# EllarBooher/Syzygy

Hardware: AMD Instinct MI355X
Metric: Mpixels/s deferred-lit+atmosphere (higher is better)
Workload: dtype f32

## Files before the change

syzygy_amd/_lib.py:

```python
import ctypes
import os
import sys

from . import abi

_HERE = os.path.dirname(os.path.abspath(__file__))
_LIB = None


class SzgError(RuntimeError):

    def __init__(self, code, message):
        super().__init__(f"szg status {code}: {message}")
        self.code = code


def library_path():
    return os.environ.get("SZG_HIP_LIBRARY") or os.path.join(_HERE, "csrc", "libszg_hip.so")


def lib():
    global _LIB
    if _LIB is None:
        path = library_path()
        if not os.path.exists(path):
            raise RuntimeError(
                f"{path} is missing: build it with `python -c 'import __graft_entry__ as g; g.build()'` "
                "(or `make -C syzygy_amd/csrc`). There is no CPU fallback for this path."
            )
        import torch

        handle = ctypes.CDLL(path)
        handle.szg_abi_version.restype = ctypes.c_int
        handle.szg_abi_version.argtypes = []
        version = handle.szg_abi_version()
        if version != abi.SZG_ABI_VERSION:
            raise RuntimeError(f"{path}: ABI version {version}, this package needs {abi.SZG_ABI_VERSION}; rebuild the library")
        abi.bind(handle, abi.ABI_FUNCTIONS)
        abi.bind(handle, abi.HOST_FUNCTIONS)
        abi.bind(handle, abi.RASTER_FUNCTIONS)
        abi.bind(handle, abi.ASSET_FUNCTIONS)
        abi.bind(handle, abi.DEBUGLINE_FUNCTIONS)
        try:
            abi.bind(handle, abi.PRESENT_FUNCTIONS)
        except AttributeError as e:
            raise RuntimeError(f"{path} predates include/szg/present.h ({e}); rebuild the library") from e
        try:
            abi.bind(handle, abi.COMPUTE_COLLECTION_FUNCTIONS)
        except AttributeError as e:
            raise RuntimeError(f"{path} predates include/szg/compute_collection.h ({e}); rebuild the library") from e
        try:
            abi.bind(handle, abi.MIPMAP_FUNCTIONS)
        except AttributeError as e:
            if "SZG_HIP_LIBRARY" not in os.environ:
                raise RuntimeError(f"{path} predates include/szg/mipmaps.h ({e}); rebuild the library") from e
            print(f"[szg] {path} predates include/szg/mipmaps.h ({e}): mip-mapped textures are unavailable with it", file=sys.stderr)
        _LIB = handle
    return _LIB


def check(status):
    if status != abi.SZG_OK:
        raise SzgError(status, lib().szg_last_error().decode("utf-8", "replace"))
    return status
```

syzygy_amd/abi.py:

```python
import ctypes as C

import numpy as np

SZG_ABI_VERSION = 2

SZG_OK = 0
SZG_ERR_INVALID_ARGUMENT = -1
SZG_ERR_NO_DEVICE = -2
SZG_ERR_OUT_OF_MEMORY = -3
SZG_ERR_HIP = -4
SZG_ERR_CAPACITY = -5

SZG_AERIAL_W = SZG_AERIAL_H = SZG_AERIAL_D = 32
SZG_OETF_PURE_GAMMA = 0
SZG_OETF_SRGB = 1

SZG_ROWTILE_COMM_ID_BYTES = 256
SZG_LUT_TRANSMITTANCE = 1
SZG_LUT_SKYVIEW = 2
SZG_FORMAT_UNDEFINED = 0
SZG_FORMAT_RGBA16_SFLOAT = 1
SZG_FORMAT_RGBA32_SFLOAT = 2
SZG_FORMAT_RGBA16_UNORM = 3
SZG_FORMAT_D32_SFLOAT = 4
# ... 481 lines not shown
    "szg_debug_lines_box_transform": (None, [P(Transform), P(AABB), P(VertexPacked)]),
}

SZG_DEBUG_LINES_CAPACITY = 1000
SZG_DEBUG_LINES_DEFAULT_WIDTH = 1.0
SZG_DEBUG_LINES_MAX_WIDTH = 256.0
SZG_DEBUG_LINES_GUARD_BAND = 16777216.0
SZG_DEBUG_LINES_MAX_CAPACITY = 1 << 24

DEBUGLINE_FUNCTIONS = {
    "szg_debug_lines_create": (C.c_int, [P(VP), U32, C.c_int]),
    "szg_debug_lines_destroy": (None, [VP]),
    "szg_debug_lines_record": (C.c_int, [VP, VP, C.c_float, Rect, P(RowTile), P(SceneTexture), U32, VP, VP, U32]),
}

SZG_PRESENT_MAX_EXTENT = 16384
SZG_FILTER_NEAREST = 0
SZG_FILTER_LINEAR = 1
SZG_PRESENT_ENCODE_NONE = 0xFFFFFFFF


class PresentInfo(C.Structure):
    _fields_ = [("src_region", Rect), ("dst_region", Rect), ("filter", U32), ("encode", U32)]


PRESENT_FUNCTIONS = {
    "szg_record_present": (C.c_int, [VP, P(Image), P(Image), P(PresentInfo)]),
}

SZG_COMPUTE_COLLECTION_SHADER_COUNT = 4
SZG_COMPUTE_COLLECTION_MAX_EXTENT = 16384
SZG_COMPUTE_COLLECTION_MAX_BLOCK_BYTES = 208
SZG_COMPUTE_COLLECTION_PREFIX_BYTES = 16
SZG_COMPUTE_COLLECTION_MAX_MEMBERS = 6
SZG_COMPUTE_COLLECTION_WORKGROUP = 16
SZG_CC_BOOLEANPUSH = 0
SZG_CC_GRADIENT_COLOR = 1
SZG_CC_SPARSE_PUSH_CONSTANT = 2
SZG_CC_MATRIX_COLOR = 3
SZG_CC_COMPONENT_FLOAT = 0
SZG_CC_COMPONENT_BOOL = 1


class CCMember(C.Structure):
    _fields_ = [("name", C.c_char_p), ("offset_bytes", U32), ("size_bytes", U32), ("padded_size_bytes", U32),
                ("component_type", U32), ("vector_width", U32), ("column_count", U32)]


class CCReflection(C.Structure):
    _fields_ = [("name", C.c_char_p), ("size_bytes", U32), ("padded_size_bytes", U32), ("layout_offset_bytes", U32),
                ("local_size", U32 * 3), ("member_count", U32), ("members", CCMember * SZG_COMPUTE_COLLECTION_MAX_MEMBERS)]


COMPUTE_COLLECTION_EXAMPLE_VALUES = {
    "booleanpush": {"row1": [1, 0, 1, 0], "row2": [0, 1, 0, 1], "row3": [1, 0, 1, 0], "row4": [0, 1, 0, 1]},
    "gradient_color": {"topColor": [0.05, 0.10, 0.60, 1.0], "bottomColor": [1.0, 0.55, 0.10, 1.0]},
    "sparse_push_constant": {"topRG": [0.9, 0.2], "topBA": [0.3, 1.0], "bottomRG": [0.1, 0.8], "bottomBA": [0.6, 1.0]},
    "matrix_color": {"red": [c / 3.0 for c in range(4) for _ in range(4)],
                     "green": [r / 3.0 for _ in range(4) for r in range(4)],
                     "blue": [((r + c) % 2) * 0.75 for c in range(4) for r in range(4)]},
}

COMPUTE_COLLECTION_FUNCTIONS = {
    "szg_compute_collection_shader_count": (U32, []),
    "szg_compute_collection_reflect": (C.c_int, [U32, P(CCReflection)]),
    "szg_record_compute_collection": (C.c_int, [VP, U32, VP, U32, P(Image), U32, U32]),
}

SZG_SAMPLER_MAX_LOD_REFERENCE = 1.0
SZG_SAMPLER_MAX_LOD_NONE = 1000.0


class TextureMips(C.Structure):
    _fields_ = [("level0_data", VP), ("d_chain", VP), ("level_count", U32)]


MIPMAP_FUNCTIONS = {
    "szg_mip_level_count": (U32, [U32, U32]),
    "szg_mip_chain_bytes": (C.c_size_t, [U32, U32]),
    "szg_record_generate_mipmaps": (C.c_int, [VP, P(Texture), VP, C.c_size_t]),
    "szg_deferred_set_texture_mips": (C.c_int, [VP, P(TextureMips), U32, C.c_float]),
}


def bind(lib, table):
    for name, (restype, argtypes) in table.items():
        fn = getattr(lib, name)
        fn.restype = restype
        fn.argtypes = argtypes
    return lib
```

syzygy_amd/csrc/api_skyview.cpp:

```cpp

#include <new>

#include "api_common.hpp"
#include "lut_state.hpp"

using namespace szg;

struct szg_skyview
{
    int device = 0;
    szg_skyview_desc desc{};
    DeviceBuffer<float> d_transmittance, d_skyview, d_multiscatter, d_aerialLuminance, d_aerialTransmittance;
    float aerialMaxDistance = 0.0f;
    mutable LutState luts;
    DeviceBuffer<unsigned> d_slutStatusAll;
    bool lutReuse = false;
    DeviceBuffer<unsigned> d_lutKey;
    DeviceBuffer<void> d_framePrep;
    DeviceBuffer<void> d_framePrepDraw;
};

static hipError_t ensure_tlut_status(szg_skyview* p, hipStream_t s)
{
    hipError_t e = hipSuccess;
    p->luts.ensure_tlut_status([&] {
        e = launch_lut_range(s, p->d_transmittance, p->desc.transmittance_width, p->desc.transmittance_height);
        return e == hipSuccess;
    });
    return e;
}

static hipError_t ensure_slut_status(szg_skyview* p, hipStream_t s)
{
    hipError_t e = hipSuccess;
    p->luts.ensure_slut_status([&] {
        e = launch_slut_check(s, p->d_skyview, p->desc.skyview_width, p->desc.skyview_height);
        return e == hipSuccess;
    });
    return e;
}

extern "C" {

int szg_skyview_create(szg_skyview_t** out, const szg_skyview_desc* desc, int device)
{
    if (out == nullptr)
    {
        return fail(SZG_ERR_INVALID_ARGUMENT, "szg_skyview_create: out is NULL");
    }
    *out = nullptr;
    szg_skyview_desc d{512u, 128u, 2048u, 1024u, 0u, 0u};
    if (desc != nullptr)
    {
        d = *desc;
    }
    if (d.transmittance_width < 2u || d.transmittance_height < 2u || d.skyview_width < 2u || d.skyview_height < 2u ||
        d.transmittance_width > 16384u || d.transmittance_height > 16384u || d.skyview_width > 16384u ||
        d.skyview_height > 16384u)
    {
        return fail(SZG_ERR_INVALID_ARGUMENT, "szg_skyview_create: LUT extents out of range");
    }
    if (d.flags != 0u)
    {
        return fail(SZG_ERR_INVALID_ARGUMENT, "szg_skyview_create: unknown flags 0x%x", d.flags);
    }
    SZG_TRY_RC(select_device(device));
    szg_skyview* p = new (std::nothrow) szg_skyview();
    if (p == nullptr)
    {
        return fail(SZG_ERR_OUT_OF_MEMORY, "szg_skyview_create: host allocation failed");
    }
    p->device = device;
    p->desc = d;
#define SZG_TRY(expr) SZG_HIP_OR(expr, szg_skyview_destroy(p), "szg_skyview_create: hipMalloc")
    size_t const aerialTexels = (size_t)SZG_AERIAL_W * SZG_AERIAL_H * SZG_AERIAL_D;
    SZG_TRY(p->d_transmittance.alloc(tlut_block_bytes(d.transmittance_width, d.transmittance_height) / sizeof(float)));
    SZG_TRY(p->d_skyview.alloc(slut_block_bytes(d.skyview_width, d.skyview_height) / sizeof(float)));
    SZG_TRY(p->d_multiscatter.alloc((size_t)SZG_MULTISCATTER_DIM * SZG_MULTISCATTER_DIM * 4u));
    SZG_TRY(p->d_aerialLuminance.alloc(aerialTexels * 4u));
    SZG_TRY(p->d_aerialTransmittance.alloc(aerialTexels * 4u));
    SZG_TRY(p->d_lutKey.alloc(LUT_KEY_DWORDS, true));
    SZG_TRY(p->d_framePrep.alloc(frame_prep_bytes()));
    SZG_TRY(p->d_slutStatusAll.alloc(SLUT_STATUS_RANKS));
    SZG_TRY(p->d_framePrepDraw.alloc(frame_prep_bytes()));
#undef SZG_TRY
    *out = p;
    return SZG_OK;
}

int szg_skyview_set_lut_reuse(szg_skyview_t* p, int enable)
{
    if (p == nullptr)
    {
        return fail(SZG_ERR_INVALID_ARGUMENT, "szg_skyview_set_lut_reuse: NULL argument");
    }
    p->lutReuse = enable != 0;
    p->luts.reuse_switched();
    return SZG_OK;
}

int szg_skyview_invalidate_luts(szg_skyview_t* p, uint32_t which)
{
    if (p == nullptr || (which & ~(SZG_LUT_TRANSMITTANCE | SZG_LUT_SKYVIEW)) != 0u)
    {
        return fail(SZG_ERR_INVALID_ARGUMENT, "szg_skyview_invalidate_luts: NULL pipeline or unknown LUT bits 0x%x", which);
    }
    if ((which & SZG_LUT_TRANSMITTANCE) != 0u)
    {
        p->luts.transmittance_exposed();
    }
    if ((which & SZG_LUT_SKYVIEW) != 0u)
    {
        p->luts.skyview_exposed();
    }
    return SZG_OK;
}

void szg_skyview_destroy(szg_skyview_t* p)
{
    if (p == nullptr)
    {
        return;
    }
    (void)hipSetDevice(p->device);
    delete p;
}

int szg_skyview_transmittance_lut(const szg_skyview_t* p, szg_image* out)
{
    if (p == nullptr || out == nullptr)
    {
        return fail(SZG_ERR_INVALID_ARGUMENT, "szg_skyview_transmittance_lut: NULL argument");
    }
    *out = make_image(p->d_transmittance, p->desc.transmittance_width, p->desc.transmittance_height, SZG_FORMAT_RGBA32_SFLOAT);
    p->luts.transmittance_exposed();
    return SZG_OK;
}

int szg_skyview_skyview_lut(const szg_skyview_t* p, szg_image* out)
{
    if (p == nullptr || out == nullptr)
    {
        return fail(SZG_ERR_INVALID_ARGUMENT, "szg_skyview_skyview_lut: NULL argument");
    }
    *out = make_image(p->d_skyview, p->desc.skyview_width, p->desc.skyview_height, SZG_FORMAT_RGBA32_SFLOAT);
    p->luts.skyview_exposed();
    return SZG_OK;
}

int szg_skyview_record_transmittance(szg_skyview_t* p, void* stream, uint32_t atmosphere_index,
                                     const szg_atmosphere_packed* d_atmospheres)
{
    if (p == nullptr || d_atmospheres == nullptr)
    {
        return fail(SZG_ERR_INVALID_ARGUMENT, "szg_skyview_record_transmittance: NULL argument");
    }
    DeviceGuard const guard(p->device);
    hipStream_t const s = static_cast<hipStream_t>(stream);
    const unsigned* dirty = nullptr;
    if (p->lutReuse)
    {
        SZG_HIP(szg::launch_lut_key(s, d_atmospheres, atmosphere_index, nullptr, 0u, p->d_lutKey, 0u, p->luts.forceTransmittance,
                                    p->d_transmittance, p->desc.transmittance_width, p->desc.transmittance_height));
        dirty = p->d_lutKey + 69;
    }
    SZG_HIP(szg::launch_transmittance(s, d_atmospheres, atmosphere_index, p->d_transmittance, p->desc.transmittance_width,
                                      p->desc.transmittance_height, dirty));
    p->luts.transmittance_recorded();
    return SZG_OK;
}

int szg_skyview_record_skyview_lut_rows(szg_skyview_t* p, void* stream, uint32_t atmosphere_index,
                                        const szg_atmosphere_packed* d_atmospheres, uint32_t view_camera_index,
                                        const szg_camera_packed* d_cameras, uint32_t row_begin, uint32_t row_end)
{
    if (p == nullptr || d_atmospheres == nullptr || d_cameras == nullptr)
    {
        return fail(SZG_ERR_INVALID_ARGUMENT, "szg_skyview_record_skyview_lut_rows: NULL argument");
    }
    if (row_begin > row_end || row_end > p->desc.skyview_height)
    {
        return fail(SZG_ERR_INVALID_ARGUMENT, "szg_skyview_record_skyview_lut_rows: rows [%u, %u) outside the %u-row LUT", row_begin,
                    row_end, p->desc.skyview_height);
    }
    DeviceGuard const guard(p->device);
    hipStream_t const s = static_cast<hipStream_t>(stream);
    bool const whole = LutState::whole(row_begin, row_end, p->desc.skyview_height);
    SZG_HIP(ensure_tlut_status(p, s));
    const unsigned* dirty = nullptr;
    if (p->lutReuse && whole)
    {
        SZG_HIP(szg::launch_lut_key(s, d_atmospheres, atmosphere_index, d_cameras, view_camera_index, p->d_lutKey, 1u, p->luts.forceSkyview,
                                    p->d_skyview, p->desc.skyview_width, p->desc.skyview_height));
        dirty = p->d_lutKey + 70;
    }
    SZG_HIP(szg::launch_frame_prep(s, d_atmospheres, atmosphere_index, p->desc.transmittance_width, p->desc.transmittance_height,
                                   p->d_framePrep));
    SZG_HIP(szg::launch_skyview(s, d_atmospheres, atmosphere_index, d_cameras, view_camera_index, p->d_transmittance,
                                p->desc.transmittance_width, p->desc.transmittance_height, p->d_skyview, p->desc.skyview_width,
                                p->desc.skyview_height, row_begin, row_end, dirty, p->d_framePrep));
    p->luts.skyview_rows_recorded(row_begin, row_end, p->desc.skyview_height);
    return SZG_OK;
}

int szg_skyview_lut_row_slice(const szg_skyview_t* p, uint32_t rank, uint32_t nranks, uint32_t* row_begin, uint32_t* row_end)
{
    if (p == nullptr || row_begin == nullptr || row_end == nullptr || nranks == 0u || rank >= nranks)
    {
        return fail(SZG_ERR_INVALID_ARGUMENT, "szg_skyview_lut_row_slice: NULL argument or rank outside [0, nranks)");
    }
    if (p->desc.skyview_height % nranks != 0u)
    {
        return fail(SZG_ERR_INVALID_ARGUMENT, "szg_skyview_lut_row_slice: %u LUT rows do not divide over %u ranks", p->desc.skyview_height,
                    nranks);
    }
    uint32_t const n = p->desc.skyview_height / nranks;
    *row_begin = rank * n;
    *row_end = (rank + 1u) * n;
    return SZG_OK;
}

int szg_skyview_allgather_lut_rows(szg_skyview_t* p, szg_rowtile_comm_t* comm, void* stream)
{
    if (p == nullptr || comm == nullptr)
    {
        return fail(SZG_ERR_INVALID_ARGUMENT, "szg_skyview_allgather_lut_rows: NULL argument");
    }
    int const nranks = szg_rowtile_comm_size(comm);
    if (nranks < 1 || p->desc.skyview_height % (uint32_t)nranks != 0u)
    {
        return fail(SZG_ERR_INVALID_ARGUMENT, "szg_skyview_allgather_lut_rows: %u LUT rows do not divide over %d ranks",
                    p->desc.skyview_height, nranks);
    }
    if (nranks > (int)szg::SLUT_STATUS_RANKS)
    {
        return fail(SZG_ERR_INVALID_ARGUMENT, "szg_skyview_allgather_lut_rows: more than %u ranks", szg::SLUT_STATUS_RANKS);
    }
    DeviceGuard const guard(p->device);
    hipStream_t const s = static_cast<hipStream_t>(stream);
    size_t const slice = (size_t)(p->desc.skyview_height / (uint32_t)nranks) * p->desc.skyview_width * 16u;
    unsigned const rank = (unsigned)szg_rowtile_comm_rank(comm);
    bool const known = p->luts.slice_status_known(rank, (uint32_t)nranks, p->desc.skyview_height);
    SZG_HIP(szg::launch_slut_status_stage(s, p->d_slutStatusAll, rank, p->d_skyview, p->desc.skyview_width,
                                          p->desc.skyview_height, known));
    int rc = szg_rowtile_allgather(comm, stream, p->d_skyview, slice);
    if (rc == SZG_OK)
    {
        rc = szg_rowtile_allgather(comm, stream, p->d_slutStatusAll, sizeof(unsigned));
    }
    if (rc == SZG_OK)
    {
        SZG_HIP(szg::launch_slut_status_reduce(s, p->d_slutStatusAll, (unsigned)nranks, p->d_skyview, p->desc.skyview_width,
                                               p->desc.skyview_height));
    }
    p->luts.rows_gathered(rc == SZG_OK);
    return rc;
}

int szg_skyview_record_skyview_lut(szg_skyview_t* p, void* stream, uint32_t atmosphere_index,
                                   const szg_atmosphere_packed* d_atmospheres, uint32_t view_camera_index,
                                   const szg_camera_packed* d_cameras)
{
    if (p == nullptr)
    {
        return fail(SZG_ERR_INVALID_ARGUMENT, "szg_skyview_record_skyview_lut: NULL argument");
    }
    return szg_skyview_record_skyview_lut_rows(p, stream, atmosphere_index, d_atmospheres, view_camera_index, d_cameras, 0u,
                                               p->desc.skyview_height);
}

static int record_composite(szg_skyview_t* p, void* stream, const szg_scene_texture* scene_texture, szg_rect draw_rect,
                            const szg_rowtile* tile, const szg_gbuffer* gbuffer, const szg_shadowmaps* shadow_maps,
                            uint32_t atmosphere_index, const szg_atmosphere_packed* d_atmospheres, uint32_t view_camera_index,
                            const szg_camera_packed* d_cameras, uint32_t sun_light_index,
                            const szg_directional_light_packed* d_lights, bool fast)
{
    if (p == nullptr || d_atmospheres == nullptr || d_cameras == nullptr || d_lights == nullptr)
    {
        return fail(SZG_ERR_INVALID_ARGUMENT, "szg_skyview_record_composite: NULL argument");
    }
    if (!check_rect(draw_rect, "szg_skyview_record_composite"))
    {
        return SZG_ERR_INVALID_ARGUMENT;
    }
// ... 139 lines not shown
```

syzygy_amd/csrc/kernels_lut.hip:

```cpp

#include "szg_device.hpp"
#include "szg_launch.hpp"

namespace szg
{
template <int CTRL> SZG_DEV float dpp(float v)
{
    return __builtin_bit_cast(float, __builtin_amdgcn_update_dpp(0, __builtin_bit_cast(int, v), CTRL, 0xF, 0xF, false));
}

constexpr int T_LANES = 8;
constexpr int T_STEPS = 500;

template <bool LEAN> SZG_DEV V3 transmittanceProduct(const Atm& a, V3 origin, V3 direction, float distance, float ndt, int sub)
{
    V3 T = splat(1.0f);
    float const rcp500 = rcpN(500.0f);
#pragma unroll 1
    for (int k = 0; k < (T_STEPS + T_LANES - 1) / T_LANES; k++)
    {
        int const i = k * T_LANES + sub;
        float const t = divRX<LEAN>(distance * ((float)i + 0.5f), 500.0f, rcp500);
        V3 const position = origin + t * direction;
        float const altitude = sqrtPX<LEAN>(dotT(position, position)) - a.planetRadius;
        Extinction const e = sampleExtinction<LEAN>(a, altitude);
        bool const valid = i < T_STEPS;
        float const fx = valid ? expX<LEAN>(ndt * e.extinction.x) : 1.0f;
        float const fy = valid ? expX<LEAN>(ndt * e.extinction.y) : 1.0f;
        float const fz = valid ? expX<LEAN>(ndt * e.extinction.z) : 1.0f;
        T.x = dpp<0x107>(T.x) * fx;
        T.y = dpp<0x107>(T.y) * fy;
        T.z = dpp<0x107>(T.z) * fz;
#pragma unroll
        for (int j = 1; j < T_LANES; j++)
        {
            T.x = dpp<0x111>(T.x) * fx;
            T.y = dpp<0x111>(T.y) * fy;
            T.z = dpp<0x111>(T.z) * fz;
        }
    }
    return T;
}

__global__ __launch_bounds__(256) void k_transmittance(const szg_atmosphere_packed* __restrict__ atmospheres,
                                                      unsigned atmosphereIndex, float4* __restrict__ lut, int W, int H,
                                                      const unsigned* __restrict__ dirty)
{
    if (dirty != nullptr && dirty[0] == 0u)
    {
        return;
    }
    int const sub = (int)(threadIdx.x & (unsigned)(T_LANES - 1));
    int const idRaw = (int)((blockIdx.x * 256u + threadIdx.x) / (unsigned)T_LANES);
    bool const inRangeTexel = idRaw < W * H;
    int const id = inRangeTexel ? idRaw : (W * H - 1);
    int const tx = id % W;
    int const ty = id / W;
    Atm const a = load_atm(atmospheres + atmosphereIndex);

    float const u = ((float)tx + 0.5f) / (float)W;
    float const v = ((float)ty + 0.5f) / (float)H;

    float const x_mu = (u - 0.5f / (float)W) / (1.0f - 1.0f / (float)W);
    float const x_radius = (v - 0.5f / (float)H) / (1.0f - 1.0f / (float)H);
    float const rho = a.H * x_radius;
    float const radius = sqrtf(rho * rho + a.Rp2);
    float const d_min = a.atmosphereRadius - radius;
    float const d_max = rho + a.H;
    float const d = (d_max - d_min) * x_mu + d_min;
    float mu = 1.0f;
    if (d != 0.0f)
    {
        mu = clampf((a.H * a.H - rho * rho - d * d) / (2.0f * radius * d), -1.0f, 1.0f);
    }

    V3 const origin = mk3(0.0f, radius, 0.0f);
    V3 const direction = mk3(sqrtf(1.0f - mu * mu), mu, 0.0f);

    float t0 = 0.0f, t1 = 0.0f;
    bool const hit = raySphere(origin, direction, a.atmosphereRadius, t0, t1);
    float const distance = hit ? t1 : 0.0f;
    float const dt = distance / 500.0f;
    float const ndt = -fabsf(dt);
    float const rmin2 = mu < 0.0f ? radius * radius * (1.0f - mu * mu) : radius * radius;
    bool const lean = waveAll(a.lean && rmin2 >= a.leanFloor2 && inRange(radius, 0x1p-30f, 0x1p30f) && inRange(distance, 0.0f, 0x1p30f));
    V3 const T = lean ? transmittanceProduct<true>(a, origin, direction, distance, ndt, sub)
                      : transmittanceProduct<false>(a, origin, direction, distance, ndt, sub);
    if (inRangeTexel && sub == T_LANES - 1)
    {
        float4 const texel = hit ? make_float4(T.x, T.y, T.z, 1.0f) : make_float4(1.0f, 1.0f, 1.0f, 1.0f);
        lut[id] = texel;
        if (!tlutTexelModerate(texel.x, texel.y, texel.z))
        {
            atomicOr(reinterpret_cast<unsigned*>(lut + (size_t)W * (size_t)H), 1u);
        }
    }
}

__global__ __launch_bounds__(256) void k_lut_range(float4* __restrict__ lut, unsigned n)
{
    unsigned const id = blockIdx.x * 256u + threadIdx.x;
    bool ok = true;
    if (id < n)
    {
        float4 const t = lut[id];
        ok = tlutTexelModerate(t.x, t.y, t.z);
    }
    if (!waveAll(ok) && (threadIdx.x & 63u) == 0u)
    {
        atomicOr(reinterpret_cast<unsigned*>(lut + n), 1u);
    }
}

__global__ __launch_bounds__(64) void k_frame_prep(const szg_atmosphere_packed* __restrict__ atmospheres, unsigned atmosphereIndex,
                                                   int tW, int tH, FramePrep* __restrict__ out,
                                                   const szg_directional_light_packed* __restrict__ sun)
{
    if (threadIdx.x != 0u)
    {
        return;
    }
    FramePrep f;
    f.a = load_atm(atmospheres + atmosphereIndex);
    f.fwidth = (float)tW;
    f.fheight = (float)tH;
    f.u_bias = 0.5f / (float)tW;
    f.u_scale = 1.0f - 1.0f / (float)tW;
    f.v_bias = 0.5f / (float)tH;
    f.v_scale = 1.0f - 1.0f / (float)tH;
    {
        auto vOf = [&](float x_radius) {
            float const t = SZG_CON(SZG_C_LUTMAP, x_radius, f.v_scale, f.v_bias);
            return SZG_CON(SZG_C_TEXCOORD, t, f.fheight, -0.5f);
        };
        float const rMax = sqrtf(f.a.innerCeil2) * (1.0f + 0x1p-16f);
        float const rhoMax = safeSqrt(rMax * rMax - f.a.Rp2);
        float const vLo = vOf(0.0f), vHi = vOf(rhoMax / f.a.H);
        bool const ok = f.a.lean && vLo >= 0.0f && floorf(vHi) + 1.0f <= f.fheight - 1.0f && vHi == vHi && tW >= 2 && tH >= 2 &&
                        (float)tW * (float)tH <= 0x1p24f;
        f.rowsInterior = ok ? 1u : 0u;
    }
#pragma unroll
    for (int k = 0; k < 16; k++)
    {
        f.sunShadow[k] = 0.0f;
    }
    if (sun != nullptr)
    {
        M4 toTex;
        float const t[16] = {0.5f, 0.0f, 0.0f, 0.0f, 0.0f, 0.5f, 0.0f, 0.0f, 0.0f, 0.0f, 1.0f, 0.0f, 0.5f, 0.5f, 0.0f, 1.0f};
#pragma unroll
        for (int k = 0; k < 16; k++)
        {
            toTex.m[k] = t[k];
        }
        M4 const sm = mul(toTex, mul(load_m4(sun->projection), load_m4(sun->view)));
#pragma unroll
        for (int k = 0; k < 16; k++)
        {
            f.sunShadow[k] = sm.m[k];
        }
    }
    *out = f;
}

__global__ __launch_bounds__(256, 4) void k_skyview(const szg_atmosphere_packed* __restrict__ atmospheres, unsigned atmosphereIndex,
                                                 const szg_camera_packed* __restrict__ cameras, unsigned cameraIndex,
                                                 const float4* __restrict__ tlut, int tW, int tH, float4* __restrict__ lut,
                                                 int W, int H, int rowBegin, int rowEnd, const unsigned* __restrict__ dirty,
                                                 const FramePrep* __restrict__ prep)
{
    if (dirty != nullptr && dirty[0] == 0u)
    {
        return;
    }
    unsigned const tid = threadIdx.x;
    unsigned const wave = tid >> 6, lane = tid & 63u;
    int const x = (int)(blockIdx.x * 32u + wave * 8u + (lane & 7u));
// ... 137 lines not shown
    {
        v = v + __shfl_xor(v, off);
    }
    return v;
}

__global__ __launch_bounds__(64) void k_multiscatter(const szg_atmosphere_packed* __restrict__ atmospheres, unsigned atmosphereIndex,
                                                     const float4* __restrict__ tlut, int tW, int tH, float4* __restrict__ out,
                                                     unsigned dim)
{
    unsigned const tx = blockIdx.x, ty = blockIdx.y, lane = threadIdx.x;
    Atm const a = load_atm(atmospheres + atmosphereIndex);
    TLut const L = make_tlut(tlut, tW, tH);
    float const PI = 3.141592653589793f;

    float const cosSunZenith = (((float)tx + 0.5f) / (float)dim) * 2.0f - 1.0f;
    float const radius = a.planetRadius + (((float)ty + 0.5f) / (float)dim) * (a.atmosphereRadius - a.planetRadius);
    V3 const sunDir = mk3(safeSqrt(1.0f - cosSunZenith * cosSunZenith), cosSunZenith, 0.0f);
    V3 const pos = mk3(0.0f, radius, 0.0f);

    float const theta = 2.0f * PI * (((float)(lane & 7u) + 0.5f) / 8.0f);
    float const cosPhi = 1.0f - 2.0f * (((float)(lane >> 3) + 0.5f) / 8.0f);
    float const sinPhi = safeSqrt(1.0f - cosPhi * cosPhi);
    V3 const dir = mk3(szg_cosf(theta) * sinPhi, cosPhi, szg_sinf(theta) * sinPhi);

    float const tMax = raycastAtmosphere(a, pos, dir);
    float gt0 = 0.0f, gt1 = 0.0f;
    bool const hitGround = raySphere(pos, dir, a.planetRadius, gt0, gt1) && gt0 > 0.0f;

    float const sin_sunRadius = szg_sinf(a.sunAngularRadius);
    float const cos_sunRadius = szg_cosf(a.sunAngularRadius);
    float const isotropic = 1.0f / (4.0f * PI);
    V3 L2 = splat(0.0f), fms = splat(0.0f), Tacc = splat(1.0f);
    float const dt = tMax / 20.0f;
    for (int i = 0; i < 20; i++)
    {
        float const t = ((float)i + 0.5f) * dt;
        V3 const p = pos + t * dir;
        float const r = length(p);
        Extinction const ex = sampleExtinction(a, r - a.planetRadius);
        V3 const sigma_s = ex.scatteringRayleigh + ex.scatteringMie;
        float const mu_s = dot(p, sunDir) / r;
        float const sin_hz = a.planetRadius / r;
        float const cos_hz = -safeSqrt(1.0f - sin_hz * sin_hz);
        V3 const T_sun = sampleT_RadiusMu(L, a, r, mu_s) * smoothstep(-sin_hz * sin_sunRadius, sin_hz * sin_sunRadius, mu_s - cos_hz * cos_sunRadius);
        V3 const T_step = mk3(szg_expf(-dt * ex.extinction.x), szg_expf(-dt * ex.extinction.y), szg_expf(-dt * ex.extinction.z));
        V3 const S = sigma_s * T_sun * isotropic;
        L2 = L2 + Tacc * ((S - S * T_step) / ex.extinction);
        fms = fms + Tacc * ((sigma_s - sigma_s * T_step) / ex.extinction);
        Tacc = Tacc * T_step;
    }
    if (hitGround)
    {
        V3 const pg = pos + tMax * dir;
        V3 const n = normalize(pg);
        float const NdotL = clampf(dot(n, sunDir), 0.0f, 1.0f);
        float const rg = length(pg);
        float const mu_g = dot(pg, sunDir) / rg;
        float const sin_hz = a.planetRadius / rg;
        float const cos_hz = -safeSqrt(1.0f - sin_hz * sin_hz);
        V3 const T_sun = sampleT_RadiusMu(L, a, rg, mu_g) * smoothstep(-sin_hz * sin_sunRadius, sin_hz * sin_sunRadius, mu_g - cos_hz * cos_sunRadius);
        L2 = L2 + Tacc * T_sun * (NdotL * (0.4f / PI));
    }
    V3 const sumL = mk3(waveSum64(L2.x), waveSum64(L2.y), waveSum64(L2.z));
    V3 const sumF = mk3(waveSum64(fms.x), waveSum64(fms.y), waveSum64(fms.z));
    if (lane == 0u)
    {
        V3 const meanL = sumL / 64.0f;
        V3 const meanF = sumF / 64.0f;
        V3 const psi = meanL / (splat(1.0f) - meanF);
        out[ty * dim + tx] = make_float4(psi.x, psi.y, psi.z, 1.0f);
    }
}

hipError_t launch_multiscatter(hipStream_t s, const szg_atmosphere_packed* d_atm, unsigned atmIndex, const float* tlut, unsigned tW,
                               unsigned tH, float* out, unsigned dim)
{
    hipLaunchKernelGGL(k_multiscatter, dim3(dim, dim), dim3(64), 0, s, d_atm, atmIndex, reinterpret_cast<const float4*>(tlut), (int)tW,
                       (int)tH, reinterpret_cast<float4*>(out), dim);
    return hipGetLastError();
}

hipError_t launch_transmittance(hipStream_t s, const szg_atmosphere_packed* d_atm, unsigned atmIndex, float* lut, unsigned W,
                                unsigned H, const unsigned* d_dirty)
{
    unsigned const n = W * H * (unsigned)T_LANES;
    if (d_dirty == nullptr)
    {
        hipError_t const e = hipMemsetAsync(lut + (size_t)W * H * 4u, 0, 4u, s);
        if (e != hipSuccess)
        {
            return e;
        }
    }
    hipLaunchKernelGGL(k_transmittance, dim3((n + 255u) / 256u), dim3(256), 0, s, d_atm, atmIndex, reinterpret_cast<float4*>(lut),
                       (int)W, (int)H, d_dirty);
    return hipGetLastError();
}

__global__ __launch_bounds__(64) void k_lut_key(const szg_atmosphere_packed* __restrict__ atmospheres, unsigned atmosphereIndex,
                                                const szg_camera_packed* __restrict__ cameras, unsigned cameraIndex,
                                                unsigned* __restrict__ state, unsigned which, unsigned force,
                                                unsigned* __restrict__ statusDword)
{
    unsigned const lane = threadIdx.x;
    const unsigned* const atm = reinterpret_cast<const unsigned*>(atmospheres + atmosphereIndex);
    unsigned* const key = state + (which == 0u ? 0u : 32u);
    bool differs = false;
    unsigned mine = 0u;
    if (lane < 32u)
    {
        mine = atm[lane];
        differs = mine != key[lane];
    }
    else if (which == 1u && lane < 35u)
    {
        mine = reinterpret_cast<const unsigned*>((cameras + cameraIndex)->position)[lane - 32u];
        differs = mine != state[64u + (lane - 32u)];
    }
    bool dirty = force != 0u || __builtin_amdgcn_ballot_w64(differs) != 0ull;
    if (which == 1u)
    {
        dirty = dirty || state[67] != state[68];
    }
    if (dirty)
    {
        if (lane < 32u)
        {
            key[lane] = mine;
        }
        else if (which == 1u && lane < 35u)
        {
            state[64u + (lane - 32u)] = mine;
        }
    }
    if (lane == 0u)
    {
        if (dirty)
        {
            if (which == 0u)
            {
                state[67] = state[67] + 1u;
            }
            else
            {
                state[68] = state[67];
            }
            statusDword[0] = 0u;
        }
        state[69u + which] = dirty ? 1u : 0u;
    }
}

hipError_t launch_lut_key(hipStream_t s, const szg_atmosphere_packed* d_atm, unsigned atmIndex, const szg_camera_packed* d_cam,
                          unsigned camIndex, unsigned* d_state, unsigned which, bool force, float* lutBlock, unsigned W, unsigned H)
{
    hipLaunchKernelGGL(k_lut_key, dim3(1), dim3(64), 0, s, d_atm, atmIndex, d_cam, camIndex, d_state, which, force ? 1u : 0u,
                       reinterpret_cast<unsigned*>(lutBlock + (size_t)W * H * 4u));
    return hipGetLastError();
}

size_t frame_prep_bytes() { return sizeof(FramePrep); }
hipError_t launch_frame_prep(hipStream_t s, const szg_atmosphere_packed* d_atm, unsigned atmIndex, unsigned tW, unsigned tH, void* d_prep,
                             const szg_directional_light_packed* d_sun)
{
    hipLaunchKernelGGL(k_frame_prep, dim3(1), dim3(64), 0, s, d_atm, atmIndex, (int)tW, (int)tH, static_cast<FramePrep*>(d_prep), d_sun);
    return hipGetLastError();
}

hipError_t launch_lut_range(hipStream_t s, float* lut, unsigned W, unsigned H)
{
    unsigned const n = W * H;
    hipError_t const e = hipMemsetAsync(lut + (size_t)n * 4u, 0, 4u, s);
    if (e != hipSuccess)
    {
        return e;
    }
    hipLaunchKernelGGL(k_lut_range, dim3((n + 255u) / 256u), dim3(256), 0, s, reinterpret_cast<float4*>(lut), n);
    return hipGetLastError();
// ... 54 lines not shown
```

syzygy_amd/csrc/szg_launch.hpp:

```cpp
#pragma once

#include <hip/hip_runtime_api.h>

#include "szg/abi.h"
#include "szg/compute_collection.h"
#include "szg/debuglines.h"
#include "szg/present.h"
#include "szg/raster.h"

namespace szg
{
struct LightRec
{
    float shadowRows[16];
    float dir[3];
    float falloffFactor;
    float colorStrength[3];
    float falloffDistance;
    float position[3];
    unsigned isSpot;
    const float* map;
    unsigned mapWidth, mapHeight;
    unsigned mapPitchFloats;
    unsigned leanOK;
    float falloffBound;
    float rcpFalloffDistance;
};
static_assert(sizeof(LightRec) == 144, "LightRec layout");

struct ShadowSlot
{
    const float* map;
    unsigned width, height, pitchFloats, pad;
};
static_assert(sizeof(ShadowSlot) == 24, "ShadowSlot layout");

struct AerialLut
{
    const float* luminance;
    unsigned W, H, D;
    float maxDistance;
};

struct TileArgs
{
    unsigned block_rows, rank, nranks, local_rows;
};

inline size_t tlut_block_bytes(unsigned W, unsigned H) { return (size_t)W * H * 16u + 16u; }
hipError_t launch_lut_range(hipStream_t s, float* lut, unsigned W, unsigned H);
hipError_t launch_transmittance(hipStream_t s, const szg_atmosphere_packed* d_atm, unsigned atmIndex, float* lut, unsigned W,
                                unsigned H, const unsigned* d_dirty = nullptr);
constexpr unsigned LUT_KEY_DWORDS = 72u;
constexpr unsigned SLUT_STATUS_RANKS = 64u;
hipError_t launch_lut_key(hipStream_t s, const szg_atmosphere_packed* d_atm, unsigned atmIndex, const szg_camera_packed* d_cam,
                          unsigned camIndex, unsigned* d_state, unsigned which, bool force, float* lutBlock, unsigned W, unsigned H);
inline size_t slut_block_bytes(unsigned W, unsigned H) { return (size_t)W * H * 16u + 16u; }
hipError_t launch_slut_check(hipStream_t s, float* lut, unsigned W, unsigned H);
hipError_t launch_slut_status_stage(hipStream_t s, unsigned* d_all, unsigned rank, const float* lut, unsigned W, unsigned H, bool known);
hipError_t launch_slut_status_reduce(hipStream_t s, const unsigned* d_all, unsigned nranks, float* lut, unsigned W, unsigned H);
hipError_t launch_skyview(hipStream_t s, const szg_atmosphere_packed* d_atm, unsigned atmIndex, const szg_camera_packed* d_cam,
                          unsigned camIndex, const float* tlut, unsigned tW, unsigned tH, float* lut, unsigned W, unsigned H,
                          unsigned rowBegin, unsigned rowEnd, const unsigned* d_dirty, const void* d_prep);
size_t frame_prep_bytes();
hipError_t launch_frame_prep(hipStream_t s, const szg_atmosphere_packed* d_atm, unsigned atmIndex, unsigned tW, unsigned tH, void* d_prep,
                             const szg_directional_light_packed* d_sun = nullptr);
hipError_t launch_light_prep(hipStream_t s, const szg_directional_light_packed* d_dir, unsigned dirCount, unsigned dirSkip,
                             const szg_spot_light_packed* d_spot, unsigned spotCount, const ShadowSlot* d_slots,
                             unsigned slotCount, LightRec* d_out);
hipError_t launch_lights(hipStream_t s, const szg_scene_texture& scene, unsigned drawW, unsigned drawH, TileArgs tile,
                         const szg_gbuffer& g, const szg_camera_packed* d_cam, unsigned camIndex, const LightRec* d_lights,
                         unsigned lightCount);
hipError_t launch_gbuffer_fill(hipStream_t s, const szg_scene_texture& scene, unsigned drawW, unsigned drawH, TileArgs tile,
                               const szg_gbuffer& g, const szg_camera_packed* d_cam, unsigned camIndex, float ground_y,
                               float ground_half_extent, float checker_cell, float ground_roughness,
                               const szg_fill_box* d_boxes, unsigned boxCount);
hipError_t launch_composite(hipStream_t s, const szg_scene_texture& scene, unsigned drawW, unsigned drawH, TileArgs tile,
                            const szg_gbuffer& g, ShadowSlot sunSlot, const szg_atmosphere_packed* d_atm, unsigned atmIndex, const szg_camera_packed* d_cam,
                            unsigned camIndex, const szg_directional_light_packed* d_dir, unsigned sunIndex, const float* tlut,
                            unsigned tW, unsigned tH, const float* slut, unsigned sW, unsigned sH, AerialLut aerial, const void* d_prep);
hipError_t launch_aerial_lut(hipStream_t s, const szg_atmosphere_packed* d_atm, unsigned atmIndex, const szg_camera_packed* d_cam,
                             unsigned camIndex, const float* tlut, unsigned tW, unsigned tH, float* luminance, float* transmittance,
                             unsigned W, unsigned H, unsigned D, float maxDistance);
hipError_t launch_multiscatter(hipStream_t s, const szg_atmosphere_packed* d_atm, unsigned atmIndex, const float* tlut, unsigned tW,
                               unsigned tH, float* out, unsigned dim);
struct ShadowGen
{
    float projView[16];
    float invProjView[16];
    float* map;
    unsigned dim, pitchFloats, pad;
};
hipError_t launch_shadow_maps(hipStream_t s, const szg_directional_light_packed* d_dir, unsigned dirCount,
                              const szg_spot_light_packed* d_spot, unsigned spotCount, const ShadowSlot* d_ownedSlots,
                              unsigned slotCount, ShadowGen* d_gen, const szg_fill_box* d_boxes, unsigned boxCount, unsigned maxDim);
hipError_t launch_shadow_prep(hipStream_t s, const szg_directional_light_packed* d_dir, unsigned dirCount,
                              const szg_spot_light_packed* d_spot, unsigned spotCount, const ShadowSlot* d_ownedSlots,
                              unsigned slotCount, ShadowGen* d_gen);

struct alignas(128) RasterDraw
{
    const szg_vertex_packed* vertices;
    const uint32_t* indices;
    const szg_mat4* models;
    const szg_mat4* mits;
    uint32_t vertexCount, firstIndex, triCount, instanceCount;
    uint32_t firstPrim;
    uint32_t pad;
    szg_texture tex[3];
    const void* mipChain[3];
    uint32_t mipLevels[3];
    float maxLod;
};
static_assert(sizeof(RasterDraw) == 256, "RasterDraw layout");
struct PrimRec
{
    float a[3], b[3], c[3];
    float z[3], w[3];
    uint32_t draw, instance, tri;
    float hx[3], hy[3], noise[3];
    float facing;
};
static_assert(sizeof(PrimRec) == 112, "PrimRec layout");
struct RasterBuffers
{
    PrimRec* prims = nullptr;
    uint2* boxes = nullptr;
    unsigned* keysA = nullptr;
    unsigned* keysB = nullptr;
    unsigned* valsA = nullptr;
    unsigned* valsB = nullptr;
    uint2* orderedBoxes = nullptr;
    uint2* chunkBoxes = nullptr;
    uint2* superBoxes = nullptr;
    void* sortTemp = nullptr;
// ... 57 lines not shown
```

syzygy_amd/pipelines.py:

```python
import ctypes as C
from collections import namedtuple

import numpy as np
import torch

from . import abi
from ._lib import check, lib


def _stream_handle(cmd):
    if cmd is None:
        return C.c_void_p(torch.cuda.current_stream().cuda_stream)
    if isinstance(cmd, torch.cuda.Stream):
        return C.c_void_p(cmd.cuda_stream)
    return C.c_void_p(int(cmd))


def _image(tensor, width, height, fmt):
    im = abi.Image()
    im.data = tensor.data_ptr()
    im.width = width
    im.height = height
    im.pitch_bytes = width * abi.TEXEL_BYTES[fmt]
    im.format = fmt
# ... 485 lines not shown
        return out


class _RawDeviceArray:
    def __init__(self, ptr, shape):
        self.__cuda_array_interface__ = {"shape": tuple(shape), "typestr": "<f4", "data": (int(ptr), False), "version": 3,
                                         "strides": None}


def _alias_tensor(ptr, shape):
    return torch.as_tensor(_RawDeviceArray(ptr, shape), device="cuda")


def _hip_memcpy2d(dst_ptr, dpitch, src_ptr, spitch, width_bytes, height):
    hip = C.CDLL("libamdhip64.so")
    hip.hipMemcpy2D.restype = C.c_int
    hip.hipMemcpy2D.argtypes = [C.c_void_p, C.c_size_t, C.c_void_p, C.c_size_t, C.c_size_t, C.c_size_t, C.c_int]
    torch.cuda.synchronize()
    rc = hip.hipMemcpy2D(dst_ptr, dpitch, src_ptr, spitch, width_bytes, height, 3)
    if rc != 0:
        raise RuntimeError(f"hipMemcpy2D failed: {rc}")


def _memcpy2d_to(im, src, rows):
    _hip_memcpy2d(im.data, im.pitch_bytes, src.data_ptr(), src.shape[1], src.shape[1], rows)


def _memcpy2d_from(im, width_bytes, rows):
    out = torch.empty((rows, width_bytes), dtype=torch.uint8, device="cuda")
    _hip_memcpy2d(out.data_ptr(), width_bytes, im.data, im.pitch_bytes, width_bytes, rows)
    return out


class SkyViewComputePipeline:

    def __init__(self, handle, desc):
        self._h = handle
        self.desc = desc

    @staticmethod
    def create(device_index=0, transmittance_extent=(512, 128), skyview_extent=(2048, 1024), flags=0):
        desc = abi.SkyviewDesc(int(transmittance_extent[0]), int(transmittance_extent[1]), int(skyview_extent[0]),
                               int(skyview_extent[1]), int(flags), 0)
        handle = C.c_void_p()
        status = lib().szg_skyview_create(C.byref(handle), C.byref(desc), int(device_index))
        if status != abi.SZG_OK:
            return None
        return SkyViewComputePipeline(handle, desc)

    def recordDrawCommands(self, cmd, sceneTexture, drawRect, gbuffer, shadowMaps, atmosphereIndex, atmospheres,
                           viewCameraIndex, cameras, sunLightIndex, lights, tile=None):
        st = sceneTexture.abi()
        check(lib().szg_skyview_record_draw_commands(
            self._h, _stream_handle(cmd), C.byref(st), drawRect, C.byref(tile) if tile is not None else None,
            C.byref(gbuffer), C.byref(shadowMaps) if shadowMaps is not None else None, int(atmosphereIndex),
            C.c_void_p(atmospheres.deviceAddress()), int(viewCameraIndex), C.c_void_p(cameras.deviceAddress()),
            int(sunLightIndex), C.c_void_p(lights.deviceAddress())))

    def recordTransmittance(self, cmd, atmosphereIndex, atmospheres):
        check(lib().szg_skyview_record_transmittance(self._h, _stream_handle(cmd), int(atmosphereIndex),
                                                     C.c_void_p(atmospheres.deviceAddress())))

    def recordSkyViewLUT(self, cmd, atmosphereIndex, atmospheres, viewCameraIndex, cameras):
        check(lib().szg_skyview_record_skyview_lut(self._h, _stream_handle(cmd), int(atmosphereIndex),
                                                   C.c_void_p(atmospheres.deviceAddress()), int(viewCameraIndex),
                                                   C.c_void_p(cameras.deviceAddress())))

    def recordSkyViewLUTRows(self, cmd, atmosphereIndex, atmospheres, viewCameraIndex, cameras, rowBegin, rowEnd):
        check(lib().szg_skyview_record_skyview_lut_rows(self._h, _stream_handle(cmd), int(atmosphereIndex),
                                                        C.c_void_p(atmospheres.deviceAddress()), int(viewCameraIndex),
                                                        C.c_void_p(cameras.deviceAddress()), int(rowBegin), int(rowEnd)))

    def lutRowSlice(self, rank, nranks):
        b, e = C.c_uint32(), C.c_uint32()
        check(lib().szg_skyview_lut_row_slice(self._h, int(rank), int(nranks), C.byref(b), C.byref(e)))
        return int(b.value), int(e.value)

    def setLUTReuse(self, enable):
        check(lib().szg_skyview_set_lut_reuse(self._h, 1 if enable else 0))

    def invalidateLUTs(self, which=abi.SZG_LUT_TRANSMITTANCE | abi.SZG_LUT_SKYVIEW):
        check(lib().szg_skyview_invalidate_luts(self._h, int(which)))

    def skyviewLUT_tensor(self):
        im = self.skyviewLUT()
        return _alias_tensor(im.data, (im.height, im.width, 4))

    def recordComposite(self, cmd, sceneTexture, drawRect, gbuffer, shadowMaps, atmosphereIndex, atmospheres, viewCameraIndex,
                        cameras, sunLightIndex, lights, tile=None):
        st = sceneTexture.abi()
        check(lib().szg_skyview_record_composite(
            self._h, _stream_handle(cmd), C.byref(st), drawRect, C.byref(tile) if tile is not None else None,
            C.byref(gbuffer), C.byref(shadowMaps) if shadowMaps is not None else None, int(atmosphereIndex),
            C.c_void_p(atmospheres.deviceAddress()), int(viewCameraIndex), C.c_void_p(cameras.deviceAddress()),
            int(sunLightIndex), C.c_void_p(lights.deviceAddress())))

    def recordMultiScatterLUT(self, cmd, atmosphereIndex, atmospheres):
        check(lib().szg_skyview_record_multiscatter_lut(self._h, _stream_handle(cmd), int(atmosphereIndex),
                                                        C.c_void_p(atmospheres.deviceAddress())))

    def multiScatterLUT(self):
        return self._lut(lib().szg_skyview_multiscatter_lut)

    def recordAerialLUT(self, cmd, atmosphereIndex, atmospheres, viewCameraIndex, cameras, maxDistanceMm):
        check(lib().szg_skyview_record_aerial_lut(self._h, _stream_handle(cmd), int(atmosphereIndex),
                                                  C.c_void_p(atmospheres.deviceAddress()), int(viewCameraIndex),
                                                  C.c_void_p(cameras.deviceAddress()), C.c_float(maxDistanceMm)))

    def recordCompositeFast(self, cmd, sceneTexture, drawRect, gbuffer, shadowMaps, atmosphereIndex, atmospheres,
                            viewCameraIndex, cameras, sunLightIndex, lights, tile=None):
        st = sceneTexture.abi()
        check(lib().szg_skyview_record_composite_fast(
            self._h, _stream_handle(cmd), C.byref(st), drawRect, C.byref(tile) if tile is not None else None,
            C.byref(gbuffer), C.byref(shadowMaps) if shadowMaps is not None else None, int(atmosphereIndex),
            C.c_void_p(atmospheres.deviceAddress()), int(viewCameraIndex), C.c_void_p(cameras.deviceAddress()),
            int(sunLightIndex), C.c_void_p(lights.deviceAddress())))

    def aerialLUT(self):
        lum, tr = abi.Image(), abi.Image()
        check(lib().szg_skyview_aerial_lut(self._h, C.byref(lum), C.byref(tr)))
        return lum, tr

    def _lut(self, getter):
        im = abi.Image()
        check(getter(self._h, C.byref(im)))
        return im

    def transmittanceLUT(self):
        return self._lut(lib().szg_skyview_transmittance_lut)

    def skyviewLUT(self):
        return self._lut(lib().szg_skyview_skyview_lut)

    def download_lut(self, im):
        raw = _memcpy2d_from(im, im.width * 16, im.height)
        return raw.cpu().numpy().view(np.float32).reshape(im.height, im.width, 4)

    def upload_lut(self, im, array):
        arr = np.ascontiguousarray(array, dtype=np.float32).reshape(im.height, im.width * 4)
        src = torch.from_numpy(arr.view(np.uint8).reshape(im.height, -1)).cuda()
        _memcpy2d_to(im, src, im.height)

    def destroy(self):
        if self._h:
            lib().szg_skyview_destroy(self._h)
            self._h = None

    def __del__(self):
        try:
            self.destroy()
        except Exception:
            pass


DrawResultsGraphics = namedtuple("DrawResultsGraphics", ["drawCalls", "verticesDrawn", "indicesDrawn"])


def _f(values, n):
    values = [float(v) for v in values]
    assert len(values) == n, values
    return (C.c_float * n)(*values)


class DebugLineGraphicsPipeline:

    def __init__(self, vertexCapacity=abi.SZG_DEBUG_LINES_CAPACITY, device_index=0):
# ... 84 lines not shown
```

Before: 2479.

## Restructure transmittance LUT product via LDS slabs and tree-reduced status flag

The transmittance kernel no longer chains an 8-lane DPP product per step. Each lane now writes its per-step extinction factors into a per-texel LDS slab, and three lanes multiply them in sequential order, two steps at a time. The separate memset and per-texel atomicOr for the LUT status word are replaced by a two-level atomic tree that publishes the status once per launch, and launch bounds now request higher occupancy. The aim is to cut the serial DPP dependency chain and a host-side memset launch, at the cost of LDS traffic, wave barriers and extra atomics. A debug status query API is also added.

```diff
diff --git a/include/szg/diagnostics.h b/include/szg/diagnostics.h
--- /dev/null
+++ b/include/szg/diagnostics.h
@@ -0,0 +1,16 @@
+#ifndef SZG_DIAGNOSTICS_H
+#define SZG_DIAGNOSTICS_H
+
+#include "szg/abi.h"
+
+#ifdef __cplusplus
+extern "C" {
+#endif
+
+int szg_skyview_debug_lut_status(const szg_skyview_t* p, void* stream, uint32_t* transmittance_status, uint32_t* skyview_status);
+
+#ifdef __cplusplus
+}
+#endif
+
+#endif
diff --git a/syzygy_amd/_lib.py b/syzygy_amd/_lib.py
--- a/syzygy_amd/_lib.py
+++ b/syzygy_amd/_lib.py
@@ -55,6 +55,11 @@
             if "SZG_HIP_LIBRARY" not in os.environ:
                 raise RuntimeError(f"{path} predates include/szg/mipmaps.h ({e}); rebuild the library") from e
             print(f"[szg] {path} predates include/szg/mipmaps.h ({e}): mip-mapped textures are unavailable with it", file=sys.stderr)
+        try:
+            abi.bind(handle, abi.DIAGNOSTIC_FUNCTIONS)
+        except AttributeError as e:
+            if "SZG_HIP_LIBRARY" not in os.environ:
+                raise RuntimeError(f"{path} predates include/szg/diagnostics.h ({e}); rebuild the library") from e
         _LIB = handle
     return _LIB
 
diff --git a/syzygy_amd/abi.py b/syzygy_amd/abi.py
--- a/syzygy_amd/abi.py
+++ b/syzygy_amd/abi.py
@@ -587,6 +587,10 @@
     "szg_deferred_set_texture_mips": (C.c_int, [VP, P(TextureMips), U32, C.c_float]),
 }
 
+DIAGNOSTIC_FUNCTIONS = {
+    "szg_skyview_debug_lut_status": (C.c_int, [VP, VP, P(U32), P(U32)]),
+}
+
 
 def bind(lib, table):
     for name, (restype, argtypes) in table.items():
diff --git a/syzygy_amd/csrc/api_skyview.cpp b/syzygy_amd/csrc/api_skyview.cpp
--- a/syzygy_amd/csrc/api_skyview.cpp
+++ b/syzygy_amd/csrc/api_skyview.cpp
@@ -3,6 +3,7 @@
 
 #include "api_common.hpp"
 #include "lut_state.hpp"
+#include "szg/diagnostics.h"
 
 using namespace szg;
 
@@ -18,6 +19,7 @@
     DeviceBuffer<unsigned> d_lutKey;
     DeviceBuffer<void> d_framePrep;
     DeviceBuffer<void> d_framePrepDraw;
+    DeviceBuffer<unsigned long long> d_tlutStatusBlock;
 };
 
 static hipError_t ensure_tlut_status(szg_skyview* p, hipStream_t s)
@@ -83,6 +85,7 @@
     SZG_TRY(p->d_framePrep.alloc(frame_prep_bytes()));
     SZG_TRY(p->d_slutStatusAll.alloc(SLUT_STATUS_RANKS));
     SZG_TRY(p->d_framePrepDraw.alloc(frame_prep_bytes()));
+    SZG_TRY(p->d_tlutStatusBlock.alloc(status_block_qwords(), true));
 #undef SZG_TRY
     *out = p;
     return SZG_OK;
@@ -165,7 +168,7 @@
         dirty = p->d_lutKey + 69;
     }
     SZG_HIP(szg::launch_transmittance(s, d_atmospheres, atmosphere_index, p->d_transmittance, p->desc.transmittance_width,
-                                      p->desc.transmittance_height, dirty));
+                                      p->desc.transmittance_height, p->d_tlutStatusBlock, dirty));
     p->luts.transmittance_recorded();
     return SZG_OK;
 }
@@ -200,6 +203,21 @@
                                 p->desc.transmittance_width, p->desc.transmittance_height, p->d_skyview, p->desc.skyview_width,
                                 p->desc.skyview_height, row_begin, row_end, dirty, p->d_framePrep));
     p->luts.skyview_rows_recorded(row_begin, row_end, p->desc.skyview_height);
+    return SZG_OK;
+}
+
+int szg_skyview_debug_lut_status(const szg_skyview_t* p, void* stream, uint32_t* transmittance_status, uint32_t* skyview_status)
+{
+    if (p == nullptr || transmittance_status == nullptr || skyview_status == nullptr)
+    {
+        return fail(SZG_ERR_INVALID_ARGUMENT, "szg_skyview_debug_lut_status: NULL argument");
+    }
+    DeviceGuard const guard(p->device);
+    SZG_HIP(hipStreamSynchronize(static_cast<hipStream_t>(stream)));
+    const float* const t = p->d_transmittance + (size_t)p->desc.transmittance_width * p->desc.transmittance_height * 4u;
+    const float* const s = p->d_skyview + (size_t)p->desc.skyview_width * p->desc.skyview_height * 4u;
+    SZG_HIP(hipMemcpy(transmittance_status, t, sizeof(uint32_t), hipMemcpyDeviceToHost));
+    SZG_HIP(hipMemcpy(skyview_status, s, sizeof(uint32_t), hipMemcpyDeviceToHost));
     return SZG_OK;
 }
 
diff --git a/syzygy_amd/csrc/kernels_lut.hip b/syzygy_amd/csrc/kernels_lut.hip
--- a/syzygy_amd/csrc/kernels_lut.hip
+++ b/syzygy_amd/csrc/kernels_lut.hip
@@ -11,45 +11,113 @@
 
 constexpr int T_LANES = 8;
 constexpr int T_STEPS = 500;
-
-template <bool LEAN> SZG_DEV V3 transmittanceProduct(const Atm& a, V3 origin, V3 direction, float distance, float ndt, int sub)
-{
-    V3 T = splat(1.0f);
+#ifndef SZG_T_BLOCK
+#define SZG_T_BLOCK 2
+#endif
+constexpr int T_BLOCK = SZG_T_BLOCK;
+constexpr int T_FULL = T_STEPS / T_LANES;
+constexpr int T_REST = T_STEPS - T_FULL * T_LANES;
+constexpr int T_TAIL = T_FULL % T_BLOCK + (T_REST != 0);
+constexpr int T_SLAB = 3 * T_LANES * T_BLOCK + 8;
+static_assert(T_REST % 4 == 0 && T_REST != 0, "the consumer reads whole float4s and the last iteration is partial");
+
+SZG_DEV void ldsOrder()
+{
+    asm volatile("" ::: "memory");
+    __builtin_amdgcn_wave_barrier();
+}
+
+template <int N> SZG_DEV float orderedProduct(float T, const float* factors)
+{
+#pragma unroll
+    for (int q = 0; q < N / 4; q++)
+    {
+        float4 const f = *reinterpret_cast<const float4*>(factors + 4 * q);
+        T = T * f.x;
+        T = T * f.y;
+        T = T * f.z;
+        T = T * f.w;
+    }
+    return T;
+}
+
+template <bool LEAN> SZG_DEV float transmittanceProduct(const Atm& a, V3 origin, V3 direction, float distance, float ndt, int sub, float* slab)
+{
+    float T = 1.0f;
     float const rcp500 = rcpN(500.0f);
-#pragma unroll 1
-    for (int k = 0; k < (T_STEPS + T_LANES - 1) / T_LANES; k++)
-    {
+    float* const mine = slab + sub;
+    const float* const channel = slab + sub * T_LANES * T_BLOCK;
+    auto factors = [&](int k, int j) {
         int const i = k * T_LANES + sub;
         float const t = divRX<LEAN>(distance * ((float)i + 0.5f), 500.0f, rcp500);
         V3 const position = origin + t * direction;
         float const altitude = sqrtPX<LEAN>(dotT(position, position)) - a.planetRadius;
         Extinction const e = sampleExtinction<LEAN>(a, altitude);
-        bool const valid = i < T_STEPS;
-        float const fx = valid ? expX<LEAN>(ndt * e.extinction.x) : 1.0f;
-        float const fy = valid ? expX<LEAN>(ndt * e.extinction.y) : 1.0f;
-        float const fz = valid ? expX<LEAN>(ndt * e.extinction.z) : 1.0f;
-        T.x = dpp<0x107>(T.x) * fx;
-        T.y = dpp<0x107>(T.y) * fy;
-        T.z = dpp<0x107>(T.z) * fz;
+        mine[0 * T_LANES * T_BLOCK + j * T_LANES] = expX<LEAN>(ndt * e.extinction.x);
+        mine[1 * T_LANES * T_BLOCK + j * T_LANES] = expX<LEAN>(ndt * e.extinction.y);
+        mine[2 * T_LANES * T_BLOCK + j * T_LANES] = expX<LEAN>(ndt * e.extinction.z);
+    };
+#pragma unroll 1
+    for (int k = 0; k < T_FULL - T_FULL % T_BLOCK; k += T_BLOCK)
+    {
 #pragma unroll
-        for (int j = 1; j < T_LANES; j++)
-        {
-            T.x = dpp<0x111>(T.x) * fx;
-            T.y = dpp<0x111>(T.y) * fy;
-            T.z = dpp<0x111>(T.z) * fz;
-        }
+        for (int j = 0; j < T_BLOCK; j++)
+        {
+            factors(k + j, j);
+        }
+        ldsOrder();
+        if (sub < 3)
+        {
+            T = orderedProduct<T_LANES * T_BLOCK>(T, channel);
+        }
+        ldsOrder();
+    }
+#pragma unroll
+    for (int j = 0; j < T_TAIL; j++)
+    {
+        factors(T_FULL - T_FULL % T_BLOCK + j, j);
+    }
+    ldsOrder();
+    if (sub < 3)
+    {
+        T = orderedProduct<T_LANES*(T_TAIL - 1) + T_REST>(T, channel);
     }
     return T;
 }
 
-__global__ __launch_bounds__(256) void k_transmittance(const szg_atmosphere_packed* __restrict__ atmospheres,
-                                                      unsigned atmosphereIndex, float4* __restrict__ lut, int W, int H,
-                                                      const unsigned* __restrict__ dirty)
+SZG_DEV void publishStatus(unsigned long long* __restrict__ block, unsigned* __restrict__ status, unsigned waveId, unsigned nWaves, bool bad)
+{
+    unsigned const leaf = waveId % STATUS_LEAVES;
+    unsigned const share = nWaves / STATUS_LEAVES + (leaf < nWaves % STATUS_LEAVES ? 1u : 0u);
+    unsigned const leaves = nWaves < STATUS_LEAVES ? nWaves : STATUS_LEAVES;
+    unsigned long long* const leafWord = block + (size_t)(1u + leaf) * STATUS_STRIDE_QWORDS;
+    unsigned long long const mine = 1ull | (bad ? 1ull << 32 : 0ull);
+    unsigned long long const leafSum = atomicAdd(leafWord, mine) + mine;
+    if ((unsigned)leafSum != share)
+    {
+        return;
+    }
+    atomicExch(leafWord, 0ull);
+    unsigned long long const up = 1ull | ((leafSum >> 32) != 0ull ? 1ull << 32 : 0ull);
+    unsigned long long const rootSum = atomicAdd(block, up) + up;
+    if ((unsigned)rootSum != leaves)
+    {
+        return;
+    }
+    atomicExch(block, 0ull);
+    status[0] = (rootSum >> 32) != 0ull ? 1u : 0u;
+}
+
+__global__ __launch_bounds__(256, 8) void k_transmittance(const szg_atmosphere_packed* __restrict__ atmospheres,
+                                                         unsigned atmosphereIndex, float4* __restrict__ lut, int W, int H,
+                                                         const unsigned* __restrict__ dirty,
+                                                         unsigned long long* __restrict__ statusBlock)
 {
     if (dirty != nullptr && dirty[0] == 0u)
     {
         return;
     }
+    __shared__ __attribute__((aligned(16))) float s_factors[256 / T_LANES][T_SLAB];
     int const sub = (int)(threadIdx.x & (unsigned)(T_LANES - 1));
     int const idRaw = (int)((blockIdx.x * 256u + threadIdx.x) / (unsigned)T_LANES);
     bool const inRangeTexel = idRaw < W * H;
@@ -84,16 +152,22 @@
     float const ndt = -fabsf(dt);
     float const rmin2 = mu < 0.0f ? radius * radius * (1.0f - mu * mu) : radius * radius;
     bool const lean = waveAll(a.lean && rmin2 >= a.leanFloor2 && inRange(radius, 0x1p-30f, 0x1p30f) && inRange(distance, 0.0f, 0x1p30f));
-    V3 const T = lean ? transmittanceProduct<true>(a, origin, direction, distance, ndt, sub)
-                      : transmittanceProduct<false>(a, origin, direction, distance, ndt, sub);
-    if (inRangeTexel && sub == T_LANES - 1)
+    float* const slab = s_factors[threadIdx.x / (unsigned)T_LANES];
+    float const Tc = lean ? transmittanceProduct<true>(a, origin, direction, distance, ndt, sub, slab)
+                          : transmittanceProduct<false>(a, origin, direction, distance, ndt, sub, slab);
+    V3 const T = mk3(Tc, dpp<0x101>(Tc), dpp<0x102>(Tc));
+    bool bad = false;
+    if (inRangeTexel && sub == 0)
     {
         float4 const texel = hit ? make_float4(T.x, T.y, T.z, 1.0f) : make_float4(1.0f, 1.0f, 1.0f, 1.0f);
         lut[id] = texel;
-        if (!tlutTexelModerate(texel.x, texel.y, texel.z))
-        {
-            atomicOr(reinterpret_cast<unsigned*>(lut + (size_t)W * (size_t)H), 1u);
-        }
+        bad = !tlutTexelModerate(texel.x, texel.y, texel.z);
+    }
+    bool const waveBad = !waveAll(!bad);
+    if ((threadIdx.x & 63u) == 0u)
+    {
+        publishStatus(statusBlock, reinterpret_cast<unsigned*>(lut + (size_t)W * (size_t)H), blockIdx.x * 4u + (threadIdx.x >> 6),
+                      gridDim.x * 4u, waveBad);
     }
 }
 
@@ -397,19 +471,11 @@
 }
 
 hipError_t launch_transmittance(hipStream_t s, const szg_atmosphere_packed* d_atm, unsigned atmIndex, float* lut, unsigned W,
-                                unsigned H, const unsigned* d_dirty)
+                                unsigned H, unsigned long long* d_statusBlock, const unsigned* d_dirty)
 {
     unsigned const n = W * H * (unsigned)T_LANES;
-    if (d_dirty == nullptr)
-    {
-        hipError_t const e = hipMemsetAsync(lut + (size_t)W * H * 4u, 0, 4u, s);
-        if (e != hipSuccess)
-        {
-            return e;
-        }
-    }
     hipLaunchKernelGGL(k_transmittance, dim3((n + 255u) / 256u), dim3(256), 0, s, d_atm, atmIndex, reinterpret_cast<float4*>(lut),
-                       (int)W, (int)H, d_dirty);
+                       (int)W, (int)H, d_dirty, d_statusBlock);
     return hipGetLastError();
 }
 
diff --git a/syzygy_amd/csrc/szg_launch.hpp b/syzygy_amd/csrc/szg_launch.hpp
--- a/syzygy_amd/csrc/szg_launch.hpp
+++ b/syzygy_amd/csrc/szg_launch.hpp
@@ -49,8 +49,11 @@
 
 inline size_t tlut_block_bytes(unsigned W, unsigned H) { return (size_t)W * H * 16u + 16u; }
 hipError_t launch_lut_range(hipStream_t s, float* lut, unsigned W, unsigned H);
+constexpr unsigned STATUS_LEAVES = 64u;
+constexpr unsigned STATUS_STRIDE_QWORDS = 16u;
+inline size_t status_block_qwords() { return (size_t)(1u + STATUS_LEAVES) * STATUS_STRIDE_QWORDS; }
 hipError_t launch_transmittance(hipStream_t s, const szg_atmosphere_packed* d_atm, unsigned atmIndex, float* lut, unsigned W,
-                                unsigned H, const unsigned* d_dirty = nullptr);
+                                unsigned H, unsigned long long* d_statusBlock, const unsigned* d_dirty = nullptr);
 constexpr unsigned LUT_KEY_DWORDS = 72u;
 constexpr unsigned SLUT_STATUS_RANKS = 64u;
 hipError_t launch_lut_key(hipStream_t s, const szg_atmosphere_packed* d_atm, unsigned atmIndex, const szg_camera_packed* d_cam,
diff --git a/syzygy_amd/pipelines.py b/syzygy_amd/pipelines.py
--- a/syzygy_amd/pipelines.py
+++ b/syzygy_amd/pipelines.py
@@ -591,6 +591,11 @@
     def invalidateLUTs(self, which=abi.SZG_LUT_TRANSMITTANCE | abi.SZG_LUT_SKYVIEW):
         check(lib().szg_skyview_invalidate_luts(self._h, int(which)))
 
+    def debugLUTStatus(self, cmd=None):
+        t, s = C.c_uint32(), C.c_uint32()
+        check(lib().szg_skyview_debug_lut_status(self._h, _stream_handle(cmd), C.byref(t), C.byref(s)))
+        return int(t.value), int(s.value)
+
     def skyviewLUT_tensor(self):
         im = self.skyviewLUT()
         return _alias_tensor(im.data, (im.height, im.width, 4))
```

Measured after the change: 2495 (median of 6 runs). About the same (+0.6%).
